# federicomegler/sq-learn

Hardware: AMD Instinct MI355X
Metric: q-means fit samples/sec (Lloyd samples*iterations/s, delta-means + tomography noise) (higher is better)
Workload: dtype fp32; 1 GPU; model=q-means k=1024 delta=0.5 (10000000 x 256 synthetic), global_batch=10000000, seq_len=256, parallelism=dp1

## Files before the change

sq_learn_amd/csrc/estep_f32.hip:

```cpp
#include "common.h"
#include "band.h"
#include "f16_tile.h"
#include "sq_api.h"

namespace sq {

constexpr int kMaxCand = 16;

#ifndef SQ_SPLIT_ACC_ALL
#define SQ_SPLIT_ACC_ALL 1
#endif
template <int KSD, int TOP = 2>
__global__ void __launch_bounds__(256, 1) estep_f32_kernel(
    const float* __restrict__ X, const _Float16* __restrict__ C, const float* __restrict__ xn,
    int* __restrict__ labels, float* __restrict__ mind, long long* __restrict__ ovf_rows,
    int* __restrict__ ovf_count, double* __restrict__ part, long long n, int k_pad, float alpha,
    float inv_alpha2, float delta_s, RngKey key, long long row_offset, int ovf_cap,
    const long long* __restrict__ rlist, const int* __restrict__ rcount,
    const float* __restrict__ cmax2_p, long long* __restrict__ mrows, int* __restrict__ mcand,
    int* __restrict__ multi_count, unsigned char* __restrict__ xflag, long long mcap) {
  const float Cm = cmax2_p ? sqrtf(*cmax2_p) * (1.0f + 0x1p-16f) : 0.0f;
  constexpr bool SPLIT_ACC = SQ_SPLIT_ACC_ALL || TOP == 3;
  constexpr float kEps3 =
      SPLIT_ACC ? (3.0f * 0x1p-22f + (KSD * 16 + 18.0f) * 0x1p-24f + 2.0f * KSD * 16 * 0x1p-34f) *
// ... 756 lines not shown
        labels[g] = -1;
      }
    }
    asm volatile("s_waitcnt lgkmcnt(0)" ::: "memory");
    __builtin_amdgcn_wave_barrier();
    }
#pragma unroll
    for (int st = 0; st < RS; ++st) xn_cur[st] = xn_nxt[st];
#if SQ_X64_STAMP
    st_post += SQ_STAMP_NOW() - sp0;
#endif
  }
  asm volatile("s_waitcnt vmcnt(0)" ::: "memory");
#if SQ_X64_STAMP
  const int sidx = blockIdx.x * NW + wave;
  if (lane == 0 && sidx < kStampWaves) {
    unsigned long long* o = g_x64_stamps + (size_t)sidx * kStampN;
    o[0] = SQ_STAMP_NOW() - st_t0; o[1] = st_sweep; o[2] = st_sync; o[3] = st_sync0;
    o[4] = st_post; o[5] = st_blocks; o[6] = st_stage; o[7] = st_cand; o[8] = st_aload;
    o[9] = st_rmin; o[10] = st_cl; o[11] = st_ub;
  }
#endif
}

constexpr int kBfLdsK = 2048;
template <int PER>
__global__ void __launch_bounds__(256) bounds_filter_kernel(
    const int* __restrict__ labels, float* __restrict__ ub, float* __restrict__ lb,
    const double* __restrict__ shift, const double* __restrict__ smax, long long n, double delta,
    long long* __restrict__ rlist, int* __restrict__ rcount, const int* __restrict__ mflag,
    long long* __restrict__ mrows, int* __restrict__ multi_count, const float* __restrict__ cc,
    const int* __restrict__ fidx, int nf, int k, int rec_on, int it_now, int it_lo,
    long long* __restrict__ mrows_b, int* __restrict__ count_b, float* __restrict__ corr,
    int* __restrict__ rec_count) {
  constexpr int kBoundsChunk = PER * 256;
  __shared__ int wsum[4], wsum_b[4];
  __shared__ int lbase[3];
  __shared__ double sf_s[65];
  __shared__ double sh_s[kBfLdsK];
  __shared__ float cm_s[kBfLdsK];
  const bool tab = k <= kBfLdsK;
  const int tid = threadIdx.x, lane = tid & 63, wv = tid >> 6;
  if (tid < nf) sf_s[tid] = shift[fidx[tid]];
  if (tab)
    for (int j = tid; j < k; j += 256) {
      sh_s[j] = shift[j];
      cm_s[j] = nf > 0 ? cc[(size_t)k * nf + j] : 0.0f;
    }
  __syncthreads();
  if (tid == 0) {
    double m = 0.0;
    for (int f = 0; f < nf; ++f) m = fmax(m, sf_s[f]);
    sf_s[nf] = m;
  }
  __syncthreads();
  const double sm = *smax;
  const long long c0 = (long long)blockIdx.x * kBoundsChunk;
  unsigned long long act = 0, rec = 0, recb = 0;
  constexpr int B = PER % 4 == 0 ? 4 : 1;
  for (int p0 = 0; p0 < PER; p0 += B) {
    int lv[B], mfv[B];
    float ubv[B], lbv[B];
    bool inb[B];
#pragma unroll
    for (int q = 0; q < B; ++q) {
      const long long i = c0 + (long long)(p0 + q) * 256 + tid;
      inb[q] = i < n;
      const long long ii = inb[q] ? i : 0;
      lv[q] = inb[q] ? labels[ii] : -1;
      if (corr && inb[q]) corr[ii] = 0.0f;
      ubv[q] = ub[ii];
      lbv[q] = lb[ii];
      mfv[q] = mflag[ii];
    }
    double shv[B];
    float cmv[B];
#pragma unroll
    for (int q = 0; q < B; ++q) {
      const int l = lv[q];
      if (tab) {
        shv[q] = l >= 0 ? sh_s[l] : 1e300;
        cmv[q] = l >= 0 ? cm_s[l] : 0.0f;
      } else {
        shv[q] = l >= 0 ? shift[l] : 1e300;
        cmv[q] = (l >= 0 && nf > 0) ? cc[(size_t)k * nf + l] : 0.0f;
      }
    }
#pragma unroll
    for (int q = 0; q < B; ++q) {
      if (!inb[q]) continue;
      const int p = p0 + q;
      const long long i = c0 + (long long)p * 256 + tid;
      const int l = lv[q];
      const double u = (double)ubv[q] + shv[q];
      auto wbound = [&](double lb0) -> double {
        double w = lb0 - sm;
        if (l >= 0 && nf > 0 && w > 0.0) {
          const double wc = fmin(w, fmax((double)cmv[q] - u, lb0 - sf_s[nf]));
          if (wc > 0.0 && wc * wc - u * u > delta * (1.0 + 1e-9) + 1e-30) {
            w = wc;
          } else {
            const float* cl = cc + (size_t)l * nf;
            if ((nf & 3) == 0) {
              for (int f = 0; f < nf; f += 4) {
                const float4 c4 = *reinterpret_cast<const float4*>(cl + f);
                w = fmin(w, fmax((double)c4.x - u, lb0 - sf_s[f]));
                w = fmin(w, fmax((double)c4.y - u, lb0 - sf_s[f + 1]));
                w = fmin(w, fmax((double)c4.z - u, lb0 - sf_s[f + 2]));
                w = fmin(w, fmax((double)c4.w - u, lb0 - sf_s[f + 3]));
              }
            } else {
              for (int f = 0; f < nf; ++f) w = fmin(w, fmax((double)cl[f] - u, lb0 - sf_s[f]));
            }
          }
        }
        return w;
      };
      const double w = wbound((double)lbv[q]);
      const bool holds = l >= 0 && w > 0.0 && w * w - u * u > delta * (1.0 + 1e-9) + 1e-30;
      if (!holds) {
        act |= 1ull << p;
      } else {
        ub[i] = (float)u * (1.0f + 0x1p-22f);
        lb[i] = (float)w * (1.0f - 0x1p-22f);
        if (mfv[q]) {
          if (rec_on && mfv[q] >= it_lo + 2 && mfv[q] <= it_now + 1) recb |= 1ull << p;
          else rec |= 1ull << p;
        }
      }
    }
  }
  const int mine = __popcll(act) | (__popcll(rec) << 16);
  const int mine_b = __popcll(recb);
  int incl = mine, incl_b = mine_b;
#pragma unroll
  for (int o = 1; o < 64; o <<= 1) {
    const int v = __shfl_up(incl, o, 64);
    const int vb = __shfl_up(incl_b, o, 64);
    if (lane >= o) {
      incl += v;
      incl_b += vb;
    }
  }
  if (lane == 63) {
    wsum[wv] = incl;
    wsum_b[wv] = incl_b;
// ... 24 lines not shown
  int mpos = lbase[1] + (ex >> 16);
  while (rec) {
    const int p = __ffsll((long long)rec) - 1;
    mrows[mpos++] = c0 + (long long)p * 256 + tid;
    rec &= rec - 1;
  }
  int bpos = lbase[2] + before_b + incl_b - mine_b;
  while (recb) {
    const int p = __ffsll((long long)recb) - 1;
    mrows_b[bpos++] = c0 + (long long)p * 256 + tid;
    recb &= recb - 1;
  }
}

struct MultiRec {
  GapRec* rec = nullptr;
  int* mflag = nullptr;
  int it_now = 0, it_lo = 0;
  int ring = 0;
  const _Float16* dsh = nullptr;
  const float* dq = nullptr;
  long long dsh_stride = 0;
  long long* mrows_b = nullptr;
  int* count_b = nullptr;
  int* n_done = nullptr;
  long long* mrows_mv = nullptr;
  int* count_mv = nullptr;
};
struct Ovf2 {
  void* rows = nullptr;
  int* count = nullptr;
};

extern "C" int sq_bounds_filter(const void* labels, void* ub, void* lb, const void* shift,
                                const void* smax, long long n, double delta, void* rlist,
                                void* rcount, const void* mflag, void* mrows, void* multi_count,
                                const void* cc, const void* fidx, int nf, int k, void* stream,
                                void* corr, void* rec_count, int rec_on, int it_now, int it_lo,
                                void* mrows_b, void* count_b) {
  if (rec_on && (it_now < 1 || it_lo < 1 || it_lo > it_now || !mrows_b || !count_b))
    return (int)hipErrorInvalidValue;
  if (n <= 0) return 0;
  if (!mflag || !mrows || !multi_count) return (int)hipErrorInvalidValue;
  if (nf < 0 || nf > 64 || (nf > 0 && (!cc || !fidx || k <= nf))) return (int)hipErrorInvalidValue;
  hipStream_t st = (hipStream_t)stream;
  static long long resident = 0;
  if (resident == 0) {
    int dev = 0, cus = 0, per_cu = 0;
    hipGetDevice(&dev);
    hipDeviceGetAttribute(&cus, hipDeviceAttributeMultiprocessorCount, dev);
    hipOccupancyMaxActiveBlocksPerMultiprocessor(&per_cu, (const void*)bounds_filter_kernel<32>,
                                                 256, 0);
    resident = (long long)(cus > 0 ? cus : 256) * (per_cu > 0 ? per_cu : 4);
  }
  auto pick = [&](int per) { return (n + per * 256LL - 1) / (per * 256LL) <= resident; };
  static const int per_env = [] {
    const char* e = getenv("SQ_BF_PER");
    return e ? atoi(e) : 0;
  }();
  int per = pick(8) ? 8 : pick(16) ? 16 : pick(20) ? 20 : pick(32) ? 32 : 64;
  if (per_env == 4 || per_env == 8 || per_env == 16 || per_env == 20 || per_env == 32 ||
      per_env == 64)
    per = per_env;
  const long long blocks = (n + per * 256LL - 1) / (per * 256LL);
  auto kern = per == 4 ? bounds_filter_kernel<4> : per == 8 ? bounds_filter_kernel<8>
            : per == 16 ? bounds_filter_kernel<16> : per == 20 ? bounds_filter_kernel<20>
            : per == 32 ? bounds_filter_kernel<32> : bounds_filter_kernel<64>;
  hipLaunchKernelGGL(kern, dim3((unsigned)blocks),
                     dim3(256), 0, st, (const int*)labels, (float*)ub, (float*)lb,
                     (const double*)shift, (const double*)smax, n, delta, (long long*)rlist,
                     (int*)rcount, (const int*)mflag, (long long*)mrows, (int*)multi_count,
                     (const float*)cc, (const int*)fidx, nf, k,
                     rec_on ? 1 : 0, it_now, it_lo, (long long*)mrows_b, (int*)count_b,
                     (float*)corr, (int*)rec_count);
  return (int)hipGetLastError();
}

__global__ void __launch_bounds__(256) fast_select_kernel(double* __restrict__ shift,
                                                          const double* __restrict__ shift_sq,
                                                          int k, int nf, int* __restrict__ idx,
                                                          double* __restrict__ smax_rest) {
  const int lane = threadIdx.x & 63;
  const int c = blockIdx.x * 4 + (threadIdx.x >> 6);
  if (c >= k) return;
  auto sv = [&](int j) -> double {
    return shift_sq ? sqrt(shift_sq[j]) * (1.0 + 1e-12) : shift[j];
  };
  const double v = sv(c);
  int rank = 0;
  for (int j = lane; j < k; j += 64) {
    const double u = sv(j);
    rank += (u > v || (u == v && j < c)) ? 1 : 0;
  }
#pragma unroll
  for (int o = 32; o > 0; o >>= 1) rank += __shfl_xor(rank, o, 64);
  if (lane == 0) {
    if (shift_sq) shift[c] = v;
    if (rank < nf) idx[rank] = c;
    if (rank == nf) *smax_rest = v > 0.0 ? v : 0.0;
  }
}

__global__ void __launch_bounds__(256) fast_cc_kernel(const float* __restrict__ C, int k, int d,
                                                      const int* __restrict__ idx, int nf,
                                                      float* __restrict__ cc) {
  __shared__ float wmin[4];
  const int lane = threadIdx.x & 63, w = threadIdx.x >> 6;
  const int j = blockIdx.x;
  float m = __builtin_inff();
  for (int f = w; f < nf; f += 4) {
    const int jf = idx[f];
    double s = 0.0;
    for (int c = lane; c < d; c += 64) {
      const double e = (double)C[(size_t)j * d + c] - (double)C[(size_t)jf * d + c];
      s = fma(e, e, s);
    }
    s = wave_sum(s);
    const float v = j == jf ? __builtin_inff() : (float)sqrt(s) * (1.0f - 0x1p-20f) - 1e-30f;
    if (lane == 0) cc[(size_t)j * nf + f] = v;
    m = fminf(m, v);
  }
  if (lane == 0) wmin[w] = m;
  __syncthreads();
  if (threadIdx.x == 0)
    cc[(size_t)k * nf + j] = fminf(fminf(wmin[0], wmin[1]), fminf(wmin[2], wmin[3]));
}

extern "C" int sq_fast_centroids(void* shift, const void* shift_sq, const void* C, int k, int d,
                                 int nf, void* idx, void* smax_rest, void* cc, void* stream) {
  if (k <= 0) return 0;
  if (nf < 0 || nf > 64 || nf >= k) return (int)hipErrorInvalidValue;
  hipStream_t st = (hipStream_t)stream;
  hipLaunchKernelGGL(fast_select_kernel, dim3((unsigned)((k + 3) / 4)), dim3(256), 0, st,
                     (double*)shift, (const double*)shift_sq, k, nf, (int*)idx,
                     (double*)smax_rest);
  if (nf > 0)
    hipLaunchKernelGGL(fast_cc_kernel, dim3((unsigned)k), dim3(256), 0, st, (const float*)C, k, d,
                       (const int*)idx, nf, (float*)cc);
  return (int)hipGetLastError();
}

template <int DX>
__global__ void __launch_bounds__(256) recheck_rows_kernel(
    const float* __restrict__ X, const float* __restrict__ Cm, const long long* __restrict__ mrows,
    const int* __restrict__ mcand, const int* __restrict__ multi_count, int* __restrict__ labels,
    float* __restrict__ mind, long long cap, double delta, RngKey key, long long row_offset,
    float* __restrict__ corr, float* __restrict__ ub, const unsigned char* __restrict__ xflag) {
  constexpr int LPR = 16;
  constexpr int FPL = DX / LPR;
  constexpr int F4 = FPL >= 4 ? FPL / 4 : 1;
  const int lane = threadIdx.x & 63;
  const int sub = lane & (LPR - 1);
  const int gbase = lane & ~(LPR - 1);
  const unsigned long long gmask = 0xffffull << gbase;
  const long long cnt = min((long long)*multi_count, cap);
  const long long gw = ((long long)blockIdx.x * blockDim.x + threadIdx.x) >> 6;
  const long long nw = ((long long)gridDim.x * blockDim.x) >> 6;
  auto cdist = [&](const float4 (&xv)[F4], int j) -> double {
    const float* cr = Cm + (size_t)j * DX;
    double s = 0.0;
#pragma unroll
    for (int q = 0; q < F4; ++q) {
      if (4 * (q * LPR + sub) < DX) {
        const float4 cv = *reinterpret_cast<const float4*>(cr + 4 * (q * LPR + sub));
        const double e0 = (double)xv[q].x - (double)cv.x, e1 = (double)xv[q].y - (double)cv.y;
        const double e2 = (double)xv[q].z - (double)cv.z, e3 = (double)xv[q].w - (double)cv.w;
        s = fma(e0, e0, fma(e1, e1, fma(e2, e2, fma(e3, e3, s))));
      }
    }
    return s;
  };
  auto process = [&](long long e, bool live) {
// ... 1107 lines not shown
```

sq_learn_amd/csrc/sq_api.h:

```cpp
#pragma once

#ifndef SQ_API
#define SQ_API
#endif

extern "C" {

SQ_API int sq_trunc_normal_add(void* x, int dtype, long long n, double b, unsigned k0, unsigned k1,
                               unsigned s0, unsigned s1, unsigned long long offset, void* stream);
SQ_API int sq_philox_normal(void* out, int dtype, long long n, double mean, double stdv,
                            unsigned k0, unsigned k1, unsigned s0, unsigned s1,
                            unsigned long long offset, void* stream);
SQ_API int sq_philox_uniform(void* out, long long n, unsigned k0, unsigned k1, unsigned s0,
                             unsigned s1, unsigned long long offset, void* stream);
SQ_API int sq_ae_batch(const void* a, const void* eps, void* out, long long n, int Q, unsigned k0,
                       unsigned k1, unsigned s0, unsigned s1, unsigned long long offset,
                       void* stream);
SQ_API int sq_pe_batch(const void* omega, const void* m, void* out, long long n, unsigned k0,
                       unsigned k1, unsigned s0, unsigned s1, unsigned long long offset,
                       void* stream);

SQ_API int sq_tomography(const void* V, int r, int d, const void* sched, int T, int mode,
                         const void* first, void* err, void* out, int norm_inf, unsigned k0,
                         unsigned k1, unsigned s0, unsigned s1, long long row_offset, void* stream,
// ... 190 lines not shown
                          const void* best_prev, int c_prev, const void* cc, int ldcc, int t,
                          long long n, long long R, int G, void* mask_out, void* surv, void* exact,
                          void* scount, void* ecount, int prune, void* stream);
SQ_API int sq_kmpp_bound(const void* Xq, int dq, const void* srow, const void* erow,
                         const void* xq2, const void* closest, const void* candq,
                         const void* cinfo, int t, int d, long long n, long long R, int G,
                         const void* surv, const void* scount, void* exact, void* ecount,
                         void* stream);
SQ_API int sq_kmpp_dots(const void* Xq, int dq, long long n, const void* candq, void* out,
                        void* stream);
SQ_API int sq_kmpp_exact(const void* X, long long ldx, int d, long long n, int t, const void* cand,
                         const void* closest, const void* w, double scale, const void* exact,
                         const void* ecount, void* mask_out, void* Dout, void* delta_part,
                         long long R, int G, void* stream);
SQ_API int sq_kmpp_pick(const void* block_tot, int G, long long R, long long n, const void* vals,
                        int t, const void* closest, const void* mask, const void* D,
                        const void* best, const void* w, double scale, void* pos, const void* X,
                        long long ldx, int d, void* cands, void* cand_ids, long long row_offset,
                        long long n_global, void* stream);
SQ_API int sq_kmpp_finish(const void* delta_part, int G, int t, void* block_tot, void* P,
                          const void* draws_next, void* vals, const void* cands,
                          const void* cand_ids, int d, void* centers, void* ids, int c,
                          void* best_out, void* stream);
SQ_API int sq_kmpp_batch(int op, const long long* ia, void* stream);

SQ_API int sq_bounds_filter(const void* labels, void* ub, void* lb, const void* shift,
                            const void* smax, long long n, double delta, void* rlist, void* rcount,
                            const void* mflag, void* mrows, void* multi_count, const void* cc,
                            const void* fidx, int nf, int k, void* stream, void* corr,
                            void* rec_count, int rec_on, int it_now, int it_lo, void* mrows_b,
                            void* count_b);
SQ_API int sq_fast_centroids(void* shift, const void* shift_sq, const void* C, int k, int d, int nf,
                             void* idx, void* smax_rest, void* cc, void* stream);
SQ_API int sq_shift_operand(const void* Cprev, const void* Cnew, int ldc, int d, int d_pad, int k,
                            double alpha, void* snap, void* dsh, void* dq, int ring, int snew,
                            unsigned valid, void* stream);
SQ_API int sq_estep_f32(const void* X, const void* C, const void* xn, void* labels, void* mind,
                        void* ovf_rows, void* ovf_count, void* part, int part_cap, void* inertia,
                        long long n, int d_pad, int k_pad, double alpha, double delta, unsigned k0,
                        unsigned k1, unsigned s0, unsigned s1, long long row_offset, int ovf_cap,
                        void* stream);
SQ_API int sq_estep_x64(const void* Xh, const void* X, const void* C, const void* Cm,
                        const void* xn, const void* cmax2, void* labels, void* mind,
                        void* dense_rows, void* ovf_rows, void* mrows, void* mcand, void* corr,
                        void* rlist, void* rcount, void* ub, void* lb, void* mflag, void* xflag,
                        void* counts, void* part, int part_cap, long long n, int d, int d_pad,
                        int k, int k_pad, double alpha, double delta, unsigned k0, unsigned k1,
                        unsigned s0, unsigned s1, long long row_offset, int list_rs, void* stream,
                        void* rec, void* rec_mflag, int it_now, int it_lo, int ring,
                        const void* dsh, const void* dq, long long dsh_stride, void* mrows_b,
                        void* count_b, void* n_done, void* mrows_mv, void* count_mv,
                        void* ovf2_rows, void* ovf2_count);
SQ_API int sq_gap_screen(const void* Xh, const void* xn, const void* mrows_b, const void* count_b,
                         const void* dsh, const void* dq, long long dsh_stride, int ring,
                         double alpha, double delta, void* labels, void* rec, void* rec_mflag,
                         int it_now, void* mrows, void* multi_count, void* n_done, void* mrows_mv,
                         void* count_mv, long long n, int d_pad, int grid_blocks, void* ydbg,
                         void* stream);
SQ_API int sq_x64_stamps(void* host, int n_waves);
SQ_API int sq_x64_stamps_clear();
SQ_API int sq_fill_mind(const void* X, int ldx, const void* Cm, int d, const void* labels,
                        void* mind, long long n, void* stream);
SQ_API int sq_sum_f32(const void* v, long long n, void* part, int extra, void* out, void* stream);
SQ_API int sq_centers_f16_operand(const void* Cm, void* op, int k, int d, int d_pad, int k_pad,
                                  double alpha, void* stream);

// ... 18 lines not shown
```

sq_learn_amd/models/cluster/_lloyd.py:

```python

import math
import os

import torch

from ...runtime.rng import RngKey
from ...ops import kmeans as K
from ...ops import linalg as L
from ...ops.random import trunc_normal_add_
from ...ops.failure import failure_inject_
from ...ops import _native as nat
from ...parallel.comm import Comm
from ...utils import tracing


class _HostScalars:

    __slots__ = ("host", "event", "sink")

    def __init__(self, host, event, sink=None):
        self.host, self.event, self.sink = host, event, sink

    def tolist(self):
        self.event.synchronize()
# ... 101 lines not shown
        self._prepare_reduce()
        self.mind_part = torch.zeros(512 + self.k, dtype=torch.float64, device=dev)
        self.incremental = (self.certified and self.sample_weight is None
                            and os.environ.get("SQ_MSTEP_INCREMENTAL", "1") != "0")
        if self.incremental:
            self.prev_labels = torch.full((self.n,), -1, dtype=torch.int32, device=dev)
            self.qsum = torch.zeros(self.k, dtype=torch.float64, device=dev)
            self.perm2 = torch.empty(max(4 * self.n, 1), dtype=torch.int32, device=dev)
            self.buf.corr = torch.zeros(max(self.n, 1), dtype=torch.float32, device=dev)
            nr = int(self._nrows_global)
            self.qexp = K.fixed_point_exp(self._max_abs ** 2 * self.dm, nr)
        self.inc_valid = False
        self.bounds = (self.certified
                       and os.environ.get("SQ_ESTEP_BOUNDS", "1") != "0")
        self.keep_max = float(os.environ.get("SQ_ESTEP_KEEP_MAX", "0.8"))
        self.probe_every = 2
        self._kept_frac = None
        self._kept_prev = None
        self._skips = 0
        self._probing = False
        self._filter_ran = False
        self._minus1 = torch.full((1,), -1, dtype=torch.int32, device=dev)
        if self.bounds:
            self.ub = torch.zeros(max(self.n, 1), dtype=torch.float32, device=dev)
            self.lb = torch.zeros(max(self.n, 1), dtype=torch.float32, device=dev)
            self.rlist = torch.empty(max(self.n, 1), dtype=torch.int64, device=dev)
            self.rcount = torch.zeros(1, dtype=torch.int32, device=dev)
            self.shift_s = torch.zeros(self.k, dtype=torch.float64, device=dev)
            self.smax = torch.zeros(1, dtype=torch.float64, device=dev)
            self.n_fast = min(int(os.environ.get("SQ_ESTEP_FAST", "16")), self.k - 1)
            self.fast_idx = torch.zeros(max(self.n_fast, 1), dtype=torch.int32, device=dev)
            self.fast_cc = torch.zeros(max(self.k * (self.n_fast + 1), 1), dtype=torch.float32,
                                       device=dev)
        self.mrec = None
        mr = os.environ.get("SQ_MULTI_RECORDS", "auto")
        if (self.bounds and self.incremental and self.d_pad % 128 == 0 and self.k <= 16384
                and (mr == "1" or (mr == "auto" and self.n >= 4_000_000))):
            R = min(max(int(os.environ.get("SQ_GAP_RING", "8")), 2), 16)
            self.mrec = torch.zeros((max(self.n, 1), 8), dtype=torch.float32, device=dev)
            self.rows_b = torch.empty(max(self.n, 1), dtype=torch.int64, device=dev)
            self.rows_moved = torch.empty(max(self.n, 1), dtype=torch.int64, device=dev)
            self.gsnap = torch.zeros((R, self.k, self.d_pad), dtype=torch.float32, device=dev)
            self.dsh = torch.zeros((R, self.k, self.d_pad), dtype=torch.float16, device=dev)
            self.dq = torch.zeros((R, self.k, 8), dtype=torch.float32, device=dev)
            self._rit = 2
            self._rlo = 2
        self.bounds_valid = False

    def _prepare_reduce(self):
        dev = self.device
        self.dm = self.Xm.shape[1]
        self.buf = K.EStepBuffers(self.n, dev)
        mx = torch.stack([self.Xm.abs().max().float() if self.n else torch.zeros((), device=dev),
                          (self.sample_weight.abs().max().float() if self.sample_weight is not None
                           and self.n else torch.zeros((), device=dev))]).double()
        nrows = torch.full((1,), float(self.n), dtype=torch.float64, device=dev)
        self.comm.all_reduce_(mx, op="max")
        self.comm.all_reduce_(nrows)
        mxl = mx.tolist()
        self._max_abs, self._nrows_global = mxl[0], nrows.item()
        self.rws = K.ReduceWorkspace(self.n, self.k, dev).set_scale(
            mxl[0], int(nrows.item()), mxl[1] if self.sample_weight is not None else None)
        self.sums = torch.zeros((self.k, self.dm), dtype=torch.float64, device=dev)
        self.counts = torch.zeros(self.k, dtype=torch.float64, device=dev)
        self.packed = torch.zeros(self.k * self.d + self.k + 1, dtype=torch.float64, device=dev)
        self.shift = torch.zeros(1, dtype=torch.float64, device=dev)
        self.shift_part = torch.zeros(self.k, dtype=torch.float64, device=dev)
        self.C = torch.zeros((self.k, self.d), dtype=torch.float32, device=dev)
        self.C_new = torch.zeros_like(self.C)
        self.cn = torch.full((self.k_pad,), K.BIG, dtype=torch.float32, device=dev)
        self.scalars = torch.zeros(4, dtype=torch.float64, device=dev)
        self.scalars[3] = -1.0
        self.weights = (self.sample_weight.to(torch.float32).contiguous()
                        if self.sample_weight is not None else None)

    def _prepare_generic(self, xn):
        self.Xf = self.X if self.X.dtype in (torch.float32, torch.float64) else self.X.float()
        self.xn = xn if xn is not None else (self.Xf * self.Xf).sum(1)
        wd = torch.float64 if self.device.type == "cpu" else torch.float32
        self.C = torch.zeros((self.k, self.d), dtype=wd, device=self.device)
# ... 43 lines not shown
        if not self.fast:
            return {}
        if self.C_op is not None:
            return {"C_op": self.C_op}
        return {"C_bf16": self.C_bf16, "cn": self.cn}

    def checkpoint_local(self):
        if getattr(self, "_ipe_lab", None) is None:
            return {}
        return {"ipe_hint": self._ipe_lab[self._ipe_cur]}

    def restore_local(self, d):
        t = d.get("ipe_hint") if d else None
        if t is None or not self.ipe:
            return
        self._ipe_buffers()
        self._ipe_lab[self._ipe_cur].copy_(t.to(self.device).to(torch.int32))
        self._ipe_hint_valid = bool((t >= 0).all())
        if getattr(self, "_ipe16", None) is not None:
            self._ipe16.invalidate_bounds()

    def _ipe_buffers(self):
        if getattr(self, "_ipe_lab", None) is None:
            self._ipe_lab = [torch.full((self.n,), -1, dtype=torch.int32, device=self.device)
                             for _ in range(2)]
            self._ipe_cur = 0
            self._ipe_xn = self.xn.float().contiguous()

    def _list_rs(self):
        force = os.environ.get("SQ_LIST_RS")
        if force is not None:
            return int(force)
        kf = self._kept_frac
        return 2 if (kf is None or kf > 0.3) else 0

    def _records_epoch(self):
        if getattr(self, "mrec", None) is not None:
            self._rit += 2
            self._rlo = self._rit

    def restore_tensors(self, d):
        self._pending = None
        self.inc_valid = False
        self.bounds_valid = False
        self._records_epoch()
        if self.fast and self.C_op is not None and "C_op" in d:
            self.C_op.copy_(d["C_op"].to(self.device))
        elif self.fast and self.C_op is None and "C_bf16" in d:
            self.C_bf16.copy_(d["C_bf16"].to(self.device))
            self.cn.copy_(d["cn"].to(self.device))

    def estep(self, C=None):
        self._pending = None
        if C is not None:
            self.set_centers(C)
        lab, mind, inertia = self._estep(self._key("band_select"), full=True)
        if self.fast and self.C_op is not None and self.certified:
            K.fill_mind_native(self.Xf32, self.C, lab, mind)
            K.sum_f32_native(mind, self.n, self.mind_part, self.buf.inertia)
        return lab, mind, inertia

    def _estep(self, key, full=False):
        self._dlists = None
        if self.fast and self.C_op is not None and self.certified:
            with tracing.range("estep_x64"):
                Cp = self.C if self.d == self.d_pad else self._padded_centers()
                rows = None
                self._filter_ran = False
                if self.bounds and not full:
                    mode = self._filter_mode()
                    if mode == "filter" and not self.bounds_valid:
                        mode = "bounds"
                else:
                    mode = "bounds" if self.bounds else "none"
                self._bounds_kept = mode != "none"
                screen = (self.incremental and not full
                          and os.environ.get("SQ_SCREEN", "1") != "0")
                records = None
                if self.mrec is not None and screen:
                    K.ensure_multi_buffers(self.buf, self.n, self.device, True)
                    R = self.dsh.shape[0]
                    records = K.multi_records(self.mrec, self.buf.mflag, self._rit,
                                              max(self._rlo, self._rit - R + 1), self.dsh,
                                              self.dq, self.rows_b, self.buf.counts[5:6],
                                              self.buf.counts[4:5], self.rows_moved,
                                              self.buf.counts[8:9])
                probe = mode == "filter" and self._probing
                zero = True
                if mode == "filter":
                    self._filter_ran = True
                    K.ensure_multi_buffers(self.buf, self.n, self.device, True)
                    self.rcount = self.buf.counts[3:4]
                    self.buf.counts.zero_()
                    K.bounds_filter_native(self.buf.labels[:self.n], self.ub, self.lb,
                                           self.shift_s, self.smax, self.delta, self.rlist,
                                           self.rcount, self.buf, cc=self.fast_cc,
                                           nf=self.n_fast, fidx=self.fast_idx, records=records)
                    if probe:
                        self.buf.counts[:3].zero_()
                        self.buf.counts[5:6].zero_()
                    else:
                        rows = (self.rlist, self.rcount)
                        self._dlists = ((self.rlist, self.rcount),
                                        (self.buf.multi_rows, self.buf.counts[7:8]),
                                        (self.rows_moved, self.buf.counts[8:9])
                                        if records is not None else None)
                    zero = False
                lab, mind = K.estep_x64_native(self.Xh16, self.Xf32, self.C_op, Cp, self.xn,
                                               self.cmax2, self.k, self.delta, self.alpha, key,
                                               self.row_offset, self.buf,
                                               bounds=(self.ub, self.lb)
                                               if self.bounds and self._bounds_kept else None,
                                               rows=rows, zero_counts=zero, screen=screen,
                                               list_rs=self._list_rs(), records=records)
                if self.mrec is not None and not screen:
                    self._records_epoch()
            return lab, mind, self.buf.inertia
        if self.fast and self.C_op is not None:
            with tracing.range("estep_f32"):
                lab, mind = K.estep_f32_native(self.Xf32, self.C_op, self.xn, self.C, self.k,
                                               self.delta, self.alpha, key, self.row_offset,
                                               self.buf)
            return lab, mind, self.buf.inertia
        if self.fast:
            with tracing.range("estep_bf16"):
                lab, mind = K.estep_native(self.Xb, self.C_bf16, self.cn, self.xn, self.k,
                                           self.delta, key, self.row_offset, self.buf)
            return lab, mind, self.buf.inertia
        if self.ipe:
            return self._estep_ipe(key)
# ... 277 lines not shown
            if self.dm == self.d:
                K.mstep_stats_native(self.sums, self.counts, self.qsum, Cold, self.k, self.dm,
                                     self.rws, self.qexp, self.buf.corr, self.n, self.mind_part,
                                     inertia, self.packed)
            else:
                K.cluster_inertia_native(self.sums, self.counts, self.qsum, Cold, self.k, self.dm,
                                         self.rws, self.qexp, self.mind_part[512:512 + self.k])
                K.sum_f32_native(self.buf.corr, self.n, self.mind_part, inertia, extra=self.k)
                K.pack_stats_native(self.sums[:, :self.d].contiguous(), self.counts, inertia,
                                    self.packed, self.k, self.d, self.rws, weighted=False)
        if events is not None:
            events[0].record()
        with tracing.range("allreduce"):
            self.comm.all_reduce_(self.packed)
        if events is not None:
            events[1].record()
        self._last_counts = self.packed[self.k * self.d:self.k * self.d + self.k]
        with tracing.range("finalize"):
            K.centroid_finalize_native(self.packed, self.C, self.C_new, self.C_bf16, self.cn,
                                       self.shift, self.k, self.d, self._noise_bound(),
                                       noise_key, self.empty_policy,
                                       shift_part=self.shift_part, scalars=self.scalars,
                                       buf=self.buf, C_f16=self.C_op, alpha=self.alpha,
                                       k_pad=self.k_pad, cmax2=self.cmax2,
                                       kept=self.rcount if self._filter_ran else self._minus1)
            self.C, self.C_new = self.C_new, self.C
            if self.intermediate_error and self.true_tomography and self.delta > 0:
                self._true_tomography_centers()
                self.scalars[1:2].copy_(((self.C.double() - self.C_new.double()) ** 2).sum())
                if self.bounds:
                    self.shift_part[:self.k].copy_(
                        ((self.C.double() - self.C_new.double()) ** 2).sum(1))
            if self.bounds and getattr(self, "_bounds_kept", True):
                if self.n_fast > 0 and self.device.type == "cuda":
                    K.fast_centroids_native(self.shift_s, self.C, self.n_fast, self.fast_idx,
                                            self.smax, self.fast_cc,
                                            shift_sq=self.shift_part[:self.k])
                else:
                    torch.sqrt(self.shift_part[:self.k], out=self.shift_s)
                    self.shift_s.mul_(1.0 + 1e-12)
                    torch.amax(self.shift_s, dim=0, keepdim=True, out=self.smax)
            if self.mrec is not None:
                R = self.dsh.shape[0]
                t = self._rit
                valid = 0
                for b in range(max(self._rlo, t + 2 - R), t + 1):
                    valid |= 1 << (b % R)
                K.shift_operand_native(self.C_new, self.C, self.alpha, self.gsnap, self.dsh,
                                       self.dq, t % R, valid)
                self._rit += 1
            if self.bounds:
                self.bounds_valid = getattr(self, "_bounds_kept", True)
        return self.scalars

    def _padded_centers(self):
        if getattr(self, "_Cpad", None) is None:
            self._Cpad = torch.zeros((self.k, self.d_pad), dtype=torch.float32, device=self.device)
        self._Cpad[:, :self.d].copy_(self.C)
        return self._Cpad

    def _true_tomography_centers(self):
        from ...quantum.device import tomography_rows_torch
        key = self._key("tomography")
        C = self.C.double()
        est = tomography_rows_torch(C, self.delta / 2.0, key, **self.tomography_kw)
        flags = (self.inc_valid, self.bounds_valid)
        self.set_centers(est.to(self.C.dtype), reset_hints=False)
# ... 120 lines not shown
```

sq_learn_amd/ops/kmeans.py:

```python

import math
import os
from typing import NamedTuple

import numpy as np

import torch

from ..runtime.rng import RngKey, philox4x32, MASK32
from . import _native as nat
from .random import amplitude_estimation_batch

FAST_D = (16, 32, 64, 128, 256)
X64_D = FAST_D + (384, 512, 640, 768, 896, 1024)
X64_MAX_K = 16384
BIG = 3.0e38


def pad_features(d):
    for f in X64_D:
        if d <= f:
            return f
    return ((d + 15) // 16) * 16

# ... 254 lines not shown

class ReduceWorkspace:

    def __init__(self, n, k, device, xexp=-30, wexp=0):
        self.hist = torch.zeros(k, dtype=torch.int32, device=device)
        self.cursor = torch.zeros(k, dtype=torch.int32, device=device)
        self.perm = torch.empty(max(n, 1), dtype=torch.int32, device=device)
        self.xexp = int(xexp)
        self.wexp = int(wexp)

    def set_scale(self, max_abs_x, n_rows, max_w=None):
        self.xexp = fixed_point_exp(max_abs_x * (max_w if max_w is not None else 1.0), n_rows)
        self.wexp = 0 if max_w is None else fixed_point_exp(max_w, n_rows)
        return self


def centroid_reduce_native(X, labels, weights, sums, counts, k, ws: ReduceWorkspace, mind=None,
                           C_old=None):
    n, d = X.shape
    assert labels.dtype == torch.int32 and sums.dtype == torch.float64 and counts.dtype == torch.float64
    assert sums.numel() >= k * d and counts.numel() >= k and labels.numel() >= n
    if mind is not None:
        assert X.dtype == torch.float32 and C_old.dtype == torch.float32
        assert tuple(C_old.shape) == (k, d) and C_old.is_contiguous() and d <= 256
    nat.native().centroid_reduce(X.data_ptr(), nat.dtype_code(X), labels.data_ptr(),
                                 0 if weights is None else weights.data_ptr(), sums.data_ptr(),
                                 counts.data_ptr(), n, d, k, ws.xexp,
                                 ws.wexp if weights is not None else 0, ws.hist.data_ptr(),
                                 ws.cursor.data_ptr(), ws.perm.data_ptr(), nat.ptr(mind),
                                 nat.ptr(C_old), nat.stream_handle(X.device))


def bounds_filter_native(labels, ub, lb, shift, smax, delta, rlist, rcount, buf: EStepBuffers,
                         cc=None, nf=0, fidx=None, records=None):
    n = labels.numel()
    assert ub.dtype == torch.float32 and lb.dtype == torch.float32 and rlist.numel() >= n
    assert shift.dtype == torch.float64 and smax.dtype == torch.float64
    assert buf.mflag is not None and buf.mflag.numel() >= n
    r = records
    nat.native().bounds_filter(labels.data_ptr(), ub.data_ptr(), lb.data_ptr(),
                               shift.data_ptr(), smax.data_ptr(), n, float(delta),
                               rlist.data_ptr(), rcount.data_ptr(), buf.mflag.data_ptr(),
                               buf.multi_rows.data_ptr(), buf.counts[2:3].data_ptr(),
                               0 if cc is None else cc.data_ptr(),
                               0 if cc is None else fidx.data_ptr(),
                               int(nf if cc is not None else 0), int(shift.numel()),
                               nat.stream_handle(labels.device),
                               0 if buf.corr is None else buf.corr.data_ptr(),
                               buf.counts[7:8].data_ptr(),
                               *((0, 0, 0, 0, 0) if r is None
                                 else (1, r.it_now, r.it_lo, r.rows_b, r.count_b)))


def fast_centroids_native(shift, C, nf, idx, smax_rest, cc, shift_sq=None):
    k, d = C.shape
    assert C.dtype == torch.float32 and C.is_contiguous() and shift.dtype == torch.float64
    assert 0 <= nf < k and idx.numel() >= nf and cc.numel() >= k * (nf + 1)
    assert shift.numel() >= k and shift.is_contiguous()
    if shift_sq is not None:
        assert shift_sq.dtype == torch.float64 and shift_sq.is_contiguous() and shift_sq.numel() >= k
    nat.native().fast_centroids(shift.data_ptr(),
                                0 if shift_sq is None else shift_sq.data_ptr(), C.data_ptr(),
                                k, d, int(nf), idx.data_ptr(), smax_rest.data_ptr(),
                                cc.data_ptr(), nat.stream_handle(C.device))


class MultiRecords(NamedTuple):
    rec: int
    mflag: int
    it_now: int
    it_lo: int
    ring: int
    dsh: int
    dq: int
    dsh_stride: int
    rows_b: int
    count_b: int
    n_done: int
    rows_moved: int
    count_moved: int


def multi_records(rec=None, mflag=None, it_now=0, it_lo=0, dsh=None, dq=None, rows_b=None,
                  count_b=None, n_done=None, rows_moved=None, count_moved=None):
    if rec is None:
        return None
    assert rec.dtype == torch.float32 and rec.shape[-1] == 8 and mflag.dtype == torch.int32
    assert dsh.dtype == torch.float16 and dq.dtype == torch.float32 and rows_b.dtype == torch.int64
    assert dsh.dim() == 3 and dq.shape[:2] == dsh.shape[:2] and dq.shape[2] == 8
    if rows_moved is not None:
        assert rows_moved.dtype == torch.int64 and rows_moved.numel() >= rows_b.numel()
        assert count_moved.dtype == torch.int32
    return MultiRecords(rec.data_ptr(), mflag.data_ptr(), int(it_now), int(it_lo),
                        int(dsh.shape[0]), dsh.data_ptr(), dq.data_ptr(), int(dsh.stride(0)),
                        rows_b.data_ptr(), count_b.data_ptr(),
                        0 if n_done is None else n_done.data_ptr(),
                        0 if rows_moved is None else rows_moved.data_ptr(),
# ... 918 lines not shown
```

Measured before the change: 16.84 billion samples*iter/s.

## Add adaptive fast-centroid set to tighten lower bounds in bounds filter

```diff
diff --git a/sq_learn_amd/csrc/estep_f32.hip b/sq_learn_amd/csrc/estep_f32.hip
--- a/sq_learn_amd/csrc/estep_f32.hip
+++ b/sq_learn_amd/csrc/estep_f32.hip
@@ -812,7 +812,7 @@
     long long* __restrict__ mrows, int* __restrict__ multi_count, const float* __restrict__ cc,
     const int* __restrict__ fidx, int nf, int k, int rec_on, int it_now, int it_lo,
     long long* __restrict__ mrows_b, int* __restrict__ count_b, float* __restrict__ corr,
-    int* __restrict__ rec_count) {
+    int* __restrict__ rec_count, const double* __restrict__ srest) {
   constexpr int kBoundsChunk = PER * 256;
   __shared__ int wsum[4], wsum_b[4];
   __shared__ int lbase[3];
@@ -835,6 +835,7 @@
   }
   __syncthreads();
   const double sm = *smax;
+  const double sr = srest ? *srest : 0.0;
   const long long c0 = (long long)blockIdx.x * kBoundsChunk;
   unsigned long long act = 0, rec = 0, recb = 0;
   constexpr int B = PER % 4 == 0 ? 4 : 1;
@@ -892,6 +893,7 @@
             } else {
               for (int f = 0; f < nf; ++f) w = fmin(w, fmax((double)cl[f] - u, lb0 - sf_s[f]));
             }
+            if (srest) w = fmin(w, fmax((double)cmv[q] - u, lb0 - sr));
           }
         }
         return w;
@@ -982,12 +984,12 @@
   int* count = nullptr;
 };
 
-extern "C" int sq_bounds_filter(const void* labels, void* ub, void* lb, const void* shift,
+static int launch_bounds_filter(const void* labels, void* ub, void* lb, const void* shift,
                                 const void* smax, long long n, double delta, void* rlist,
                                 void* rcount, const void* mflag, void* mrows, void* multi_count,
                                 const void* cc, const void* fidx, int nf, int k, void* stream,
                                 void* corr, void* rec_count, int rec_on, int it_now, int it_lo,
-                                void* mrows_b, void* count_b) {
+                                void* mrows_b, void* count_b, const void* srest) {
   if (rec_on && (it_now < 1 || it_lo < 1 || it_lo > it_now || !mrows_b || !count_b))
     return (int)hipErrorInvalidValue;
   if (n <= 0) return 0;
@@ -1022,53 +1024,116 @@
                      (int*)rcount, (const int*)mflag, (long long*)mrows, (int*)multi_count,
                      (const float*)cc, (const int*)fidx, nf, k,
                      rec_on ? 1 : 0, it_now, it_lo, (long long*)mrows_b, (int*)count_b,
-                     (float*)corr, (int*)rec_count);
+                     (float*)corr, (int*)rec_count, (const double*)srest);
   return (int)hipGetLastError();
+}
+
+extern "C" int sq_bounds_filter(const void* labels, void* ub, void* lb, const void* shift,
+                                const void* smax, long long n, double delta, void* rlist,
+                                void* rcount, const void* mflag, void* mrows, void* multi_count,
+                                const void* cc, const void* fidx, int nf, int k, void* stream,
+                                void* corr, void* rec_count, int rec_on, int it_now, int it_lo,
+                                void* mrows_b, void* count_b) {
+  return launch_bounds_filter(labels, ub, lb, shift, smax, n, delta, rlist, rcount, mflag, mrows,
+                              multi_count, cc, fidx, nf, k, stream, corr, rec_count, rec_on, it_now,
+                              it_lo, mrows_b, count_b, nullptr);
+}
+
+extern "C" int sq_bounds_filter_adaptive(const void* labels, void* ub, void* lb, const void* shift,
+                                         const void* smax, long long n, double delta, void* rlist,
+                                         void* rcount, const void* mflag, void* mrows,
+                                         void* multi_count, const void* cc, const void* fidx,
+                                         int nf, int k, void* stream, void* corr, void* rec_count,
+                                         int rec_on, int it_now, int it_lo, void* mrows_b,
+                                         void* count_b, const void* fast) {
+  if (!fast || nf <= 0) return (int)hipErrorInvalidValue;
+  return launch_bounds_filter(labels, ub, lb, shift, smax, n, delta, rlist, rcount, mflag, mrows,
+                              multi_count, cc, fidx, nf, k, stream, corr, rec_count, rec_on, it_now,
+                              it_lo, mrows_b, count_b, fast);
 }
 
 __global__ void __launch_bounds__(256) fast_select_kernel(double* __restrict__ shift,
                                                           const double* __restrict__ shift_sq,
-                                                          int k, int nf, int* __restrict__ idx,
-                                                          double* __restrict__ smax_rest) {
+                                                          int k, int nf, int cap,
+                                                          int* __restrict__ idx,
+                                                          double* __restrict__ smax_rest,
+                                                          double* __restrict__ sorted) {
   const int lane = threadIdx.x & 63;
   const int c = blockIdx.x * 4 + (threadIdx.x >> 6);
   if (c >= k) return;
-  auto sv = [&](int j) -> double {
-    return shift_sq ? sqrt(shift_sq[j]) * (1.0 + 1e-12) : shift[j];
-  };
-  const double v = sv(c);
+  const double* key = shift_sq ? shift_sq : shift;
+  const double v = key[c];
   int rank = 0;
   for (int j = lane; j < k; j += 64) {
-    const double u = sv(j);
+    const double u = key[j];
     rank += (u > v || (u == v && j < c)) ? 1 : 0;
   }
 #pragma unroll
   for (int o = 32; o > 0; o >>= 1) rank += __shfl_xor(rank, o, 64);
   if (lane == 0) {
-    if (shift_sq) shift[c] = v;
-    if (rank < nf) idx[rank] = c;
-    if (rank == nf) *smax_rest = v > 0.0 ? v : 0.0;
+    const double s = shift_sq ? sqrt(v) * (1.0 + 1e-12) : v;
+    if (shift_sq) shift[c] = s;
+    if (rank < cap) idx[rank] = c;
+    if (sorted) {
+      if (rank <= cap) sorted[rank] = s;
+    } else if (rank == nf) {
+      *smax_rest = s > 0.0 ? s : 0.0;
+    }
   }
 }
 
 __global__ void __launch_bounds__(256) fast_cc_kernel(const float* __restrict__ C, int k, int d,
                                                       const int* __restrict__ idx, int nf,
-                                                      float* __restrict__ cc) {
+                                                      float* __restrict__ cc,
+                                                      const double* __restrict__ sorted, int cap,
+                                                      double thr, int* __restrict__ nfd,
+                                                      double* __restrict__ smax_rest,
+                                                      double* __restrict__ fast) {
   __shared__ float wmin[4];
+  __shared__ int wcnt[4];
   const int lane = threadIdx.x & 63, w = threadIdx.x >> 6;
   const int j = blockIdx.x;
+  int nF = nf;
+  if (sorted) {
+    const double t = thr * sorted[cap];
+    int cnt = 0;
+    for (int r = threadIdx.x; r < cap; r += 256) cnt += sorted[r] > t ? 1 : 0;
+#pragma unroll
+    for (int o = 32; o > 0; o >>= 1) cnt += __shfl_xor(cnt, o, 64);
+    if (lane == 0) wcnt[w] = cnt;
+    __syncthreads();
+    nF = min(max(wcnt[0] + wcnt[1] + wcnt[2] + wcnt[3], nf), cap);
+    if (j == 0 && threadIdx.x == 0) {
+      *nfd = nF;
+      *smax_rest = fmax(sorted[nF], 0.0);
+      fast[0] = fmax(sorted[nf], 0.0);
+      fast[1] = t;
+    }
+  }
   float m = __builtin_inff();
-  for (int f = w; f < nf; f += 4) {
-    const int jf = idx[f];
-    double s = 0.0;
+  for (int f0 = 4 * w; f0 < nF; f0 += 16) {
+    int jf[4];
+    double s[4] = {0.0, 0.0, 0.0, 0.0};
+#pragma unroll
+    for (int q = 0; q < 4; ++q) jf[q] = idx[min(f0 + q, nF - 1)];
     for (int c = lane; c < d; c += 64) {
-      const double e = (double)C[(size_t)j * d + c] - (double)C[(size_t)jf * d + c];
-      s = fma(e, e, s);
-    }
-    s = wave_sum(s);
-    const float v = j == jf ? __builtin_inff() : (float)sqrt(s) * (1.0f - 0x1p-20f) - 1e-30f;
-    if (lane == 0) cc[(size_t)j * nf + f] = v;
-    m = fminf(m, v);
+      const double x = (double)C[(size_t)j * d + c];
+#pragma unroll
+      for (int q = 0; q < 4; ++q) {
+        const double e = x - (double)C[(size_t)jf[q] * d + c];
+        s[q] = fma(e, e, s[q]);
+      }
+    }
+#pragma unroll
+    for (int q = 0; q < 4; ++q) s[q] = wave_sum(s[q]);
+#pragma unroll
+    for (int q = 0; q < 4; ++q) {
+      if (f0 + q >= nF) continue;
+      const float v =
+          j == jf[q] ? __builtin_inff() : (float)sqrt(s[q]) * (1.0f - 0x1p-20f) - 1e-30f;
+      if (lane == 0 && f0 + q < nf) cc[(size_t)j * nf + f0 + q] = v;
+      m = fminf(m, v);
+    }
   }
   if (lane == 0) wmin[w] = m;
   __syncthreads();
@@ -1076,18 +1141,38 @@
     cc[(size_t)k * nf + j] = fminf(fminf(wmin[0], wmin[1]), fminf(wmin[2], wmin[3]));
 }
 
+static int launch_fast_centroids(void* shift, const void* shift_sq, const void* C, int k, int d,
+                                 int nf, void* idx, void* smax_rest, void* cc, void* stream,
+                                 double thr, void* sorted, int cap, void* nfd, void* fast) {
+  hipStream_t st = (hipStream_t)stream;
+  hipLaunchKernelGGL(fast_select_kernel, dim3((unsigned)((k + 3) / 4)), dim3(256), 0, st,
+                     (double*)shift, (const double*)shift_sq, k, nf, cap, (int*)idx,
+                     (double*)smax_rest, (double*)sorted);
+  if (nf > 0)
+    hipLaunchKernelGGL(fast_cc_kernel, dim3((unsigned)k), dim3(256), 0, st, (const float*)C, k, d,
+                       (const int*)idx, nf, (float*)cc, (const double*)sorted, cap, thr,
+                       (int*)nfd, (double*)smax_rest, (double*)fast);
+  return (int)hipGetLastError();
+}
+
 extern "C" int sq_fast_centroids(void* shift, const void* shift_sq, const void* C, int k, int d,
                                  int nf, void* idx, void* smax_rest, void* cc, void* stream) {
   if (k <= 0) return 0;
   if (nf < 0 || nf > 64 || nf >= k) return (int)hipErrorInvalidValue;
-  hipStream_t st = (hipStream_t)stream;
-  hipLaunchKernelGGL(fast_select_kernel, dim3((unsigned)((k + 3) / 4)), dim3(256), 0, st,
-                     (double*)shift, (const double*)shift_sq, k, nf, (int*)idx,
-                     (double*)smax_rest);
-  if (nf > 0)
-    hipLaunchKernelGGL(fast_cc_kernel, dim3((unsigned)k), dim3(256), 0, st, (const float*)C, k, d,
-                       (const int*)idx, nf, (float*)cc);
-  return (int)hipGetLastError();
+  return launch_fast_centroids(shift, shift_sq, C, k, d, nf, idx, smax_rest, cc, stream, 0.0,
+                               nullptr, nf, nullptr, nullptr);
+}
+
+extern "C" int sq_fast_centroids_adaptive(void* shift, const void* shift_sq, const void* C, int k,
+                                          int d, int nf, double thr, void* idx, void* sorted,
+                                          void* nfd, void* fast, void* smax_rest, void* cc,
+                                          void* stream) {
+  if (k <= 0) return 0;
+  if (nf < 1 || nf > 64 || nf >= k || !(thr >= 0.0) || !idx || !sorted || !nfd || !fast)
+    return (int)hipErrorInvalidValue;
+  const int cap = nf > k / 2 ? nf : k / 2;
+  return launch_fast_centroids(shift, shift_sq, C, k, d, nf, idx, smax_rest, cc, stream, thr,
+                               sorted, cap, nfd, fast);
 }
 
 template <int DX>
diff --git a/sq_learn_amd/csrc/sq_api.h b/sq_learn_amd/csrc/sq_api.h
--- a/sq_learn_amd/csrc/sq_api.h
+++ b/sq_learn_amd/csrc/sq_api.h
@@ -246,6 +246,16 @@
                             void* count_b);
 SQ_API int sq_fast_centroids(void* shift, const void* shift_sq, const void* C, int k, int d, int nf,
                              void* idx, void* smax_rest, void* cc, void* stream);
+SQ_API int sq_fast_centroids_adaptive(void* shift, const void* shift_sq, const void* C, int k, int d,
+                                      int nf, double thr, void* idx, void* sorted, void* nfd,
+                                      void* fast, void* smax_rest, void* cc, void* stream);
+SQ_API int sq_bounds_filter_adaptive(const void* labels, void* ub, void* lb, const void* shift,
+                                     const void* smax, long long n, double delta, void* rlist,
+                                     void* rcount, const void* mflag, void* mrows,
+                                     void* multi_count, const void* cc, const void* fidx, int nf,
+                                     int k, void* stream, void* corr, void* rec_count, int rec_on,
+                                     int it_now, int it_lo, void* mrows_b, void* count_b,
+                                     const void* fast);
 SQ_API int sq_shift_operand(const void* Cprev, const void* Cnew, int ldc, int d, int d_pad, int k,
                             double alpha, void* snap, void* dsh, void* dq, int ring, int snew,
                             unsigned valid, void* stream);
diff --git a/sq_learn_amd/models/cluster/_lloyd.py b/sq_learn_amd/models/cluster/_lloyd.py
--- a/sq_learn_amd/models/cluster/_lloyd.py
+++ b/sq_learn_amd/models/cluster/_lloyd.py
@@ -157,6 +157,15 @@
             self.fast_idx = torch.zeros(max(self.n_fast, 1), dtype=torch.int32, device=dev)
             self.fast_cc = torch.zeros(max(self.k * (self.n_fast + 1), 1), dtype=torch.float32,
                                        device=dev)
+            self.fast_adapt = (os.environ.get("SQ_ESTEP_FAST_ADAPT", "1") != "0"
+                               and self.n_fast > 0 and dev.type == "cuda")
+            self.fast_set = None
+            if self.fast_adapt:
+                self.fast_set = K.fast_set(
+                    self.k, self.n_fast, float(os.environ.get("SQ_ESTEP_FAST_THR", "32")), dev)
+                self.fast_idx = self.fast_set.idx
+                self.fast_nf = self.fast_set.size
+                self.fast_aux = self.fast_set.rest
         self.mrec = None
         mr = os.environ.get("SQ_MULTI_RECORDS", "auto")
         if (self.bounds and self.incremental and self.d_pad % 128 == 0 and self.k <= 16384
@@ -171,6 +180,9 @@
             self._rit = 2
             self._rlo = 2
         self.bounds_valid = False
+        self._list_rs_len = 0
+        if dev.type == "cuda" and os.environ.get("SQ_LIST_RS_LEN", "1") != "0":
+            self._list_rs_len = torch.cuda.get_device_properties(dev).multi_processor_count
 
     def _prepare_reduce(self):
         dev = self.device
@@ -280,7 +292,12 @@
         if force is not None:
             return int(force)
         kf = self._kept_frac
-        return 2 if (kf is None or kf > 0.3) else 0
+        if kf is None or kf > 0.3:
+            return 2
+        rows, rnd = kf * self.n, 128 * self._list_rs_len
+        if self._list_rs_len and rnd < rows <= 2 * rnd:
+            return 2
+        return 0
 
     def _records_epoch(self):
         if getattr(self, "mrec", None) is not None:
@@ -343,7 +360,8 @@
                     K.bounds_filter_native(self.buf.labels[:self.n], self.ub, self.lb,
                                            self.shift_s, self.smax, self.delta, self.rlist,
                                            self.rcount, self.buf, cc=self.fast_cc,
-                                           nf=self.n_fast, fidx=self.fast_idx, records=records)
+                                           nf=self.n_fast, fidx=self.fast_idx, records=records,
+                                           fast=self.fast_set)
                     if probe:
                         self.buf.counts[:3].zero_()
                         self.buf.counts[5:6].zero_()
@@ -687,7 +705,11 @@
                     self.shift_part[:self.k].copy_(
                         ((self.C.double() - self.C_new.double()) ** 2).sum(1))
             if self.bounds and getattr(self, "_bounds_kept", True):
-                if self.n_fast > 0 and self.device.type == "cuda":
+                if self.fast_set is not None:
+                    K.fast_centroids_adaptive_native(self.shift_s, self.C, self.fast_set,
+                                                     self.smax, self.fast_cc,
+                                                     shift_sq=self.shift_part[:self.k])
+                elif self.n_fast > 0 and self.device.type == "cuda":
                     K.fast_centroids_native(self.shift_s, self.C, self.n_fast, self.fast_idx,
                                             self.smax, self.fast_cc,
                                             shift_sq=self.shift_part[:self.k])
diff --git a/sq_learn_amd/ops/kmeans.py b/sq_learn_amd/ops/kmeans.py
--- a/sq_learn_amd/ops/kmeans.py
+++ b/sq_learn_amd/ops/kmeans.py
@@ -310,12 +310,28 @@
 
 
 def bounds_filter_native(labels, ub, lb, shift, smax, delta, rlist, rcount, buf: EStepBuffers,
-                         cc=None, nf=0, fidx=None, records=None):
+                         cc=None, nf=0, fidx=None, records=None, fast=None):
     n = labels.numel()
     assert ub.dtype == torch.float32 and lb.dtype == torch.float32 and rlist.numel() >= n
     assert shift.dtype == torch.float64 and smax.dtype == torch.float64
     assert buf.mflag is not None and buf.mflag.numel() >= n
     r = records
+    if fast is not None:
+        assert cc is not None and cc.numel() >= shift.numel() * (fast.nf + 1)
+        p = lambda a: a or None
+        rc = _adaptive_entries()[1](
+            labels.data_ptr(), ub.data_ptr(), lb.data_ptr(), shift.data_ptr(), smax.data_ptr(), n,
+            float(delta), rlist.data_ptr(), rcount.data_ptr(), buf.mflag.data_ptr(),
+            buf.multi_rows.data_ptr(), buf.counts[2:3].data_ptr(), cc.data_ptr(),
+            fast.idx.data_ptr(), fast.nf, int(shift.numel()),
+            p(nat.stream_handle(labels.device)),
+            p(0 if buf.corr is None else buf.corr.data_ptr()), buf.counts[7:8].data_ptr(),
+            *((0, 0, 0, None, None) if r is None
+              else (1, r.it_now, r.it_lo, r.rows_b, r.count_b)),
+            fast.rest.data_ptr())
+        if rc != 0:
+            raise RuntimeError(f"sq_learn_amd native launch failed: sq_bounds_filter_adaptive ({rc})")
+        return
     nat.native().bounds_filter(labels.data_ptr(), ub.data_ptr(), lb.data_ptr(),
                                shift.data_ptr(), smax.data_ptr(), n, float(delta),
                                rlist.data_ptr(), rcount.data_ptr(), buf.mflag.data_ptr(),
@@ -341,6 +357,59 @@
                                 0 if shift_sq is None else shift_sq.data_ptr(), C.data_ptr(),
                                 k, d, int(nf), idx.data_ptr(), smax_rest.data_ptr(),
                                 cc.data_ptr(), nat.stream_handle(C.device))
+
+
+_ADAPTIVE = None
+
+
+def _adaptive_entries():
+    global _ADAPTIVE
+    if _ADAPTIVE is None:
+        import ctypes
+        P, L, I, D = ctypes.c_void_p, ctypes.c_longlong, ctypes.c_int, ctypes.c_double
+        lib = ctypes.CDLL(nat.loaded_path())
+        fc, bf = lib.sq_fast_centroids_adaptive, lib.sq_bounds_filter_adaptive
+        fc.restype = bf.restype = I
+        fc.argtypes = [P, P, P, I, I, I, D, P, P, P, P, P, P, P]
+        bf.argtypes = [P, P, P, P, P, L, D, P, P, P, P, P, P, P, I, I, P, P, P, I, I, I, P, P, P]
+        _ADAPTIVE = (fc, bf)
+    return _ADAPTIVE
+
+
+class FastSet(NamedTuple):
+    nf: int
+    thr: float
+    idx: torch.Tensor
+    sorted: torch.Tensor
+    size: torch.Tensor
+    rest: torch.Tensor
+
+
+def fast_set(k, nf, thr, device):
+    cap = max(int(nf), k // 2)
+    return FastSet(int(nf), float(thr),
+                   torch.zeros(cap, dtype=torch.int32, device=device),
+                   torch.zeros(cap + 1, dtype=torch.float64, device=device),
+                   torch.zeros(1, dtype=torch.int32, device=device),
+                   torch.zeros(2, dtype=torch.float64, device=device))
+
+
+def fast_centroids_adaptive_native(shift, C, fs: FastSet, smax_rest, cc, shift_sq=None):
+    k, d = C.shape
+    nf = fs.nf
+    assert C.dtype == torch.float32 and C.is_contiguous() and shift.dtype == torch.float64
+    assert 1 <= nf < k and nf <= 64 and cc.numel() >= k * (nf + 1)
+    assert fs.idx.numel() >= max(nf, k // 2) and fs.sorted.numel() >= max(nf, k // 2) + 1
+    assert shift.numel() >= k and shift.is_contiguous()
+    if shift_sq is not None:
+        assert shift_sq.dtype == torch.float64 and shift_sq.is_contiguous() and shift_sq.numel() >= k
+    p = lambda a: a or None
+    rc = _adaptive_entries()[0](
+        shift.data_ptr(), p(0 if shift_sq is None else shift_sq.data_ptr()), C.data_ptr(), k, d,
+        nf, fs.thr, fs.idx.data_ptr(), fs.sorted.data_ptr(), fs.size.data_ptr(),
+        fs.rest.data_ptr(), smax_rest.data_ptr(), cc.data_ptr(), p(nat.stream_handle(C.device)))
+    if rc != 0:
+        raise RuntimeError(f"sq_learn_amd native launch failed: sq_fast_centroids_adaptive ({rc})")
 
 
 class MultiRecords(NamedTuple):
```

Result: no change. 16.87 billion samples*iter/s (median of 6 runs) (+0.2%).
